# AutoAILab/FusionDepth

Hardware: AMD Instinct MI355X
Metric: training images/sec (640x192, ResNet-18, 4-beam) (higher is better)
Workload: dtype f32

## Files before the change

fusiondepth_amd/csrc/conv_wino.hip:

```cpp
#include "../../include/fdhip.h"
#include "fd_common.h"
#include "conv_fast.h"
#include "conv_limb.h"
#include <stdlib.h>
#include <type_traits>

namespace {

typedef float f32x16 __attribute__((ext_vector_type(16)));
typedef float f32x2 __attribute__((ext_vector_type(2)));
typedef unsigned int u32x2 __attribute__((__vector_size__(2 * sizeof(unsigned int))));

__device__ __forceinline__ f32x2 fd_ldg64(__amdgpu_buffer_rsrc_t r, unsigned byte_off) {
    return __builtin_bit_cast(f32x2, __builtin_amdgcn_raw_buffer_load_b64(r, (int)byte_off, 0, 0));
}
__device__ __attribute__((noinline)) float wino_act_slow(float v, int act) {
    if (act == 2) return v > 0.f ? v : expm1f(v);
    if (act == 3) return 1.0f / (1.0f + expf(-v));
    return tanhf(v);
}
__device__ __forceinline__ float wino_act(float v, int act) {
    if (act >= 2) return wino_act_slow(v, act);
    return act == 1 ? fmaxf(v, 0.f) : v;
}
// ... 1538 lines not shown
            rx[i].z = fmaf(x_sgn, rz[i].z, rx[i].z); rx[i].w = fmaf(x_sgn, rz[i].w, rx[i].w);
        }
        if (!HALFM || i < 2) *reinterpret_cast<f32x2*>(qa) = ra[i];
        const bool L = rf & 1, R = rf & 2;
        float4 d;
        d.y = L ? rx[i].x : rx[i].y;
        d.z = L ? rx[i].y : rx[i].z;
        d.w = L ? rx[i].z : rx[i].w;
        d.x = L ? (refl ? d.z : 0.f) : rx[i].x;
        d.w = R ? (refl ? d.y : 0.f) : d.w;
        *reinterpret_cast<float4*>(smem + buf * WG_BUF_FLOATS + WBM * LDG + (rw + 16 * i) * LDX + 4 * p) = d;
    };

    const int wm = wave >> 1, wn = wave & 1;
    const int arow = lane >> 5, acol = lane & 31;
    f32x16 acc[4];
#pragma unroll
    for (int t = 0; t < 4; ++t)
#pragma unroll
        for (int r = 0; r < 16; ++r) acc[t][r] = 0.f;

    constexpr int NK = WGP / 2, LS = NK / 2;
    constexpr int NKW = HALFM ? NK / 2 : NK;
    static_assert(!HALFM || NKW == LS, "HALFM: the four row loads / stores of a chunk sit in its four k-steps");
    const int kb = HALFM ? wm * NKW : 0;
    if (nchunk > 0) {
        prep_chunk(true);
        rf = pf;
#pragma unroll
        for (int i = 0; i < 4; ++i) load_row(i);
#pragma unroll
        for (int i = 0; i < 4; ++i) store_row(0, i);
        prep_chunk(1 < nchunk);
        rf = pf;
#pragma unroll
        for (int i = 0; i < 4; ++i) load_row(i);
        prep_chunk(2 < nchunk);
        __syncthreads();
        for (int ch = 0; ch < nchunk; ++ch) {
            const int cur = ch & 1;
            const float* pa = smem + cur * WG_BUF_FLOATS + ((HALFM ? 0 : 32 * wm) + acol) * LDG + 2 * arow + 4 * kb;
            const float* pb = smem + cur * WG_BUF_FLOATS + WBM * LDG + (32 * wn + acol) * LDX + 4 * arow + 8 * kb;
            float av[2][4], bv[2][4];
            f32x2 yy;
            float4 dd;
            auto read_ops = [&](int kk2) __attribute__((always_inline)) {
                yy = *reinterpret_cast<const f32x2*>(pa + 4 * kk2);
                dd = *reinterpret_cast<const float4*>(pb + 8 * kk2);
            };
            auto xform = [&](int nb) __attribute__((always_inline)) {
                av[nb][0] = yy.x; av[nb][1] = yy.x + yy.y; av[nb][2] = yy.x - yy.y; av[nb][3] = yy.y;
                bv[nb][0] = dd.x - dd.z; bv[nb][1] = dd.y + dd.z; bv[nb][2] = dd.z - dd.y; bv[nb][3] = dd.y - dd.w;
            };
            read_ops(0); xform(0);
#pragma unroll
            for (int kk = 0; kk < NKW; ++kk) {
                const int cb = kk & 1, nb = cb ^ 1;
                __builtin_amdgcn_sched_barrier(0);
                acc[0] = __builtin_amdgcn_mfma_f32_32x32x2f32(av[cb][0], bv[cb][0], acc[0], 0, 0, 0);
                __builtin_amdgcn_sched_barrier(0);
                if (kk + 1 < NKW) read_ops(kk + 1);
                __builtin_amdgcn_sched_barrier(0);
                acc[1] = __builtin_amdgcn_mfma_f32_32x32x2f32(av[cb][1], bv[cb][1], acc[1], 0, 0, 0);
                __builtin_amdgcn_sched_barrier(0);
                if (kk < LS) store_row(cur ^ 1, kk);
                __builtin_amdgcn_sched_barrier(0);
                acc[2] = __builtin_amdgcn_mfma_f32_32x32x2f32(av[cb][2], bv[cb][2], acc[2], 0, 0, 0);
                __builtin_amdgcn_sched_barrier(0);
                if (kk + 1 < NKW) xform(nb);
                __builtin_amdgcn_sched_barrier(0);
                acc[3] = __builtin_amdgcn_mfma_f32_32x32x2f32(av[cb][3], bv[cb][3], acc[3], 0, 0, 0);
                __builtin_amdgcn_sched_barrier(0);
                if (kk < LS) load_row(kk);
                if (kk == (HALFM ? NKW - 1 : LS)) rf = pf;
                if (kk == NKW - 1) prep_chunk(ch + 3 < nchunk);
            }
            __builtin_amdgcn_sched_barrier(0);
            __syncthreads();
        }
    }

    if constexpr (HALFM) {
        float* red = smem + ((wn * 64) << 6) + lane;
        if (wm == 1) {
#pragma unroll
            for (int t = 0; t < 4; ++t)
#pragma unroll
                for (int r = 0; r < 16; ++r) red[(t * 16 + r) << 6] = acc[t][r];
        }
        __syncthreads();
        if (wm == 1) return;
#pragma unroll
        for (int t = 0; t < 4; ++t)
#pragma unroll
            for (int r = 0; r < 16; ++r) acc[t][r] += red[(t * 16 + r) << 6];
    }
    const int c = c0 + 32 * wn + acol;
    const __amdgpu_buffer_rsrc_t rsS = fd_make_rsrc(g.slabs + (size_t)bs * ((size_t)g.M * (3 * R) * g.C));
    const int mb = m0 + (HALFM ? 0 : 32 * wm) + 4 * arow;
    const unsigned col = (c < g.C) ? 4u * (unsigned)(ky * 3 * g.C + c) : FD_OOB;
    const unsigned row_step = 4u * (3u * R) * (unsigned)g.C, kx_step = 4u * (unsigned)g.C;
#pragma unroll
    for (int r = 0; r < 16; ++r) {
        const int m = mb + (r & 3) + 8 * (r >> 2);
        const unsigned off = (m < g.M) ? col + (unsigned)m * row_step : FD_OOB;
        const float M0 = acc[0][r], M1 = acc[1][r], M2 = acc[2][r], M3 = acc[3][r];
        const float h = 0.5f * (M1 + M2);
        __builtin_amdgcn_raw_buffer_store_b32(__builtin_bit_cast(unsigned, M0 + h), rsS, (int)off, 0, 0);
        __builtin_amdgcn_raw_buffer_store_b32(__builtin_bit_cast(unsigned, 0.5f * (M1 - M2)), rsS, (int)(off + kx_step), 0, 0);
        __builtin_amdgcn_raw_buffer_store_b32(__builtin_bit_cast(unsigned, h - M3), rsS, (int)(off + 2u * kx_step), 0, 0);
    }
}

constexpr int WL_HPL = 64 * 16 + 64;
constexpr int WL_PLANE = 2 * WL_HPL;
constexpr int WL_OP = 12 * WL_PLANE;
constexpr int WL_LDS_BYTES = 2 * WL_OP;


template <bool REFL>
__global__ void __launch_bounds__(WNT) k_wgrad_wino_limb(WinoWgradArgs g) {
    extern __shared__ __attribute__((aligned(16))) float smem[];
    unsigned char* smemb = reinterpret_cast<unsigned char*>(smem);
    const int tid = threadIdx.x, lane = tid & 63;
    const int wave = __builtin_amdgcn_readfirstlane(tid >> 6);
    const int W2 = g.W >> 1;
    const int HT = g.H >> 1;
    constexpr int R = 4;
    const int plane2 = HT * W2, Np = g.Nb * plane2;
    const unsigned hw = (unsigned)(g.H * g.W);
    const int ctiles = (g.C + WBN - 1) / WBN;
    int bt, bs, by;
    if (g.slice_major == 2) {
        const int mtiles = (g.M + WBM - 1) / WBM, nt = R * ctiles * mtiles;
        const int L = blockIdx.x, xcd = L & 7, k = L >> 3;
        int t;
        if (g.xcds_per_slice <= 1) { t = k % nt; bs = (k / nt) * 8 + xcd; }
        else { const int per = nt / g.xcds_per_slice; bs = xcd / g.xcds_per_slice; t = (xcd % g.xcds_per_slice) * per + k; }
        by = t / (R * ctiles);
        bt = t - by * R * ctiles;
    } else {
        bt = g.slice_major ? blockIdx.z : blockIdx.x; bs = g.slice_major ? blockIdx.x : blockIdx.z; by = blockIdx.y;
    }
    const int ky = bt / ctiles, c0 = (bt - ky * ctiles) * WBN;
    const int m0 = by * WBM;
    const int pp_lo = (int)((long)bs * g.pairs_per_split < Np ? (long)bs * g.pairs_per_split : Np);
    const int pp_hi = (long)pp_lo + g.pairs_per_split < Np ? pp_lo + (int)g.pairs_per_split : Np;
    const int nchunk = pp_hi > pp_lo ? (pp_hi - pp_lo + WGP - 1) / WGP : 0;

    const int q = tid & 3, row = tid >> 2;
    unsigned a_row, b_row;
    {
        int m = m0 + row; m = m < g.M ? m : g.M - 1;
        int c = c0 + row; c = c < g.C ? c : g.C - 1;
        a_row = 4u * (unsigned)m * hw; b_row = 4u * (unsigned)c * hw;
    }
    const __amdgpu_buffer_rsrc_t rsY = fd_make_rsrc(g.dY);
    const __amdgpu_buffer_rsrc_t rsX = __builtin_amdgcn_make_buffer_rsrc(const_cast<float*>(g.X), 0, (int)(4u * (unsigned)g.Nb * (unsigned)g.C * hw), 0x00020000);
    float4 ya[1][2], yb[1][2];
    float4 xa[1][2], xb[1][2];
    f32x2 xa2[1], xb2[1];
    unsigned a_off = FD_OOB, x_off = FD_OOB, a_off2 = FD_OOB, x_off2 = FD_OOB;
    const int yr_a = ky == 3 ? 1 : 0;
    const bool y_two = ky == 1 || ky == 2;
    const float y_sgn = ky == 2 ? -1.f : 1.f;
    const int xr_a = ky == 0 ? 0 : (ky == 2 ? 2 : 1), xr_b = ky == 3 ? 3 : (ky == 2 ? 1 : 2);
    const float x_sgn = ky == 1 ? 1.f : -1.f;
    int pf = 0, rf = 0;
    int pc = pp_lo;
    int cn, cy, cj;
    {
        const int pq = pp_lo + 4 * q;
        cn = pq / plane2;
        const int rem = pq - cn * plane2;
        cy = rem / W2; cj = rem - cy * W2;
    }
    auto prep_chunk = [&](bool live) __attribute__((always_inline)) {
        const int pg = pc + 4 * q;
        const bool ok = live & (pg < pp_hi);
        const int n = cn, y = cy, j = cj;
        const bool e_left = j == 0, e_right = 2 * j + 8 >= g.W;
        auto x_row = [&](int r) __attribute__((always_inline)) {
            const bool inb = (unsigned)r < (unsigned)g.H;
            int rr_ = r < 0 ? -r : r;
            rr_ = rr_ >= g.H ? 2 * g.H - 2 - rr_ : rr_;
            const int ruse = REFL ? rr_ : r;
            const bool okb = ok & (REFL | inb);
            const unsigned base = 4u * ((unsigned)n * (unsigned)g.C * hw + (unsigned)(ruse * g.W + 2 * j));
            return okb ? (e_left ? base : base - 4u) : FD_OOB;
        };
        const unsigned yo = 4u * ((unsigned)n * (unsigned)g.M * hw + (unsigned)((2 * y + yr_a) * g.W + 2 * j));
        a_off = ok ? yo : FD_OOB;
        a_off2 = (ok & y_two) ? yo + 4u * (unsigned)g.W : FD_OOB;
        x_off = x_row(2 * y - 1 + xr_a);
        x_off2 = x_row(2 * y - 1 + xr_b);
        pf = (e_left ? 1 : 0) | (e_right ? 2 : 0);
        pc += WGP;
        cj += g.adv_j;
        const bool c1 = cj >= W2;
        cj -= c1 ? W2 : 0;
        cy += g.adv_y + (c1 ? 1 : 0);
        const bool c2 = cy >= HT;
        cy -= c2 ? HT : 0;
        cn += g.adv_n + (c2 ? 1 : 0);
    };
    auto load_all = [&](auto slot_tag) __attribute__((always_inline)) {
        constexpr int S = decltype(slot_tag)::value;
        ya[S][0] = fd_ldg128(rsY, a_off + a_row); ya[S][1] = fd_ldg128(rsY, a_off + a_row + 16u);
        yb[S][0] = fd_ldg128(rsY, a_off2 + a_row); yb[S][1] = fd_ldg128(rsY, a_off2 + a_row + 16u);
        xa[S][0] = fd_ldg128(rsX, x_off + b_row); xa[S][1] = fd_ldg128(rsX, x_off + b_row + 16u); xa2[S] = fd_ldg64(rsX, x_off + b_row + 32u);
        xb[S][0] = fd_ldg128(rsX, x_off2 + b_row); xb[S][1] = fd_ldg128(rsX, x_off2 + b_row + 16u); xb2[S] = fd_ldg64(rsX, x_off2 + b_row + 32u);
    };
    unsigned char* const slot = smemb + (q >> 1) * WL_HPL + row * 16 + 8 * (q & 1);
    auto store_all = [&](auto slot_tag) __attribute__((always_inline)) {
        constexpr int S = decltype(slot_tag)::value;
        float Y[8], X[10];
        Y[0] = fmaf(y_sgn, yb[S][0].x, ya[S][0].x); Y[1] = fmaf(y_sgn, yb[S][0].y, ya[S][0].y); Y[2] = fmaf(y_sgn, yb[S][0].z, ya[S][0].z); Y[3] = fmaf(y_sgn, yb[S][0].w, ya[S][0].w);
        Y[4] = fmaf(y_sgn, yb[S][1].x, ya[S][1].x); Y[5] = fmaf(y_sgn, yb[S][1].y, ya[S][1].y); Y[6] = fmaf(y_sgn, yb[S][1].z, ya[S][1].z); Y[7] = fmaf(y_sgn, yb[S][1].w, ya[S][1].w);
        float r[10];
        r[0] = fmaf(x_sgn, xb[S][0].x, xa[S][0].x); r[1] = fmaf(x_sgn, xb[S][0].y, xa[S][0].y); r[2] = fmaf(x_sgn, xb[S][0].z, xa[S][0].z); r[3] = fmaf(x_sgn, xb[S][0].w, xa[S][0].w);
        r[4] = fmaf(x_sgn, xb[S][1].x, xa[S][1].x); r[5] = fmaf(x_sgn, xb[S][1].y, xa[S][1].y); r[6] = fmaf(x_sgn, xb[S][1].z, xa[S][1].z); r[7] = fmaf(x_sgn, xb[S][1].w, xa[S][1].w);
        r[8] = fmaf(x_sgn, xb2[S].x, xa2[S].x); r[9] = fmaf(x_sgn, xb2[S].y, xa2[S].y);
        const bool L = rf & 1, Rr = rf & 2;
#pragma unroll
        for (int k = 1; k < 10; ++k) X[k] = L ? r[k - 1] : r[k];
        X[0] = L ? (REFL ? X[2] : 0.f) : r[0];
        X[9] = Rr ? (REFL ? X[7] : 0.f) : X[9];
        unsigned char* qa = slot;
        unsigned char* qb = slot + WL_OP;
#pragma unroll
        for (int t = 0; t < 4; ++t) {
            float pv[4], qv[4];
#pragma unroll
            for (int k = 0; k < 4; ++k) {
                const float y0 = Y[2 * k], y1 = Y[2 * k + 1];
                const float d0 = X[2 * k], d1 = X[2 * k + 1], d2 = X[2 * k + 2], d3 = X[2 * k + 3];
                pv[k] = t == 0 ? y0 : (t == 1 ? y0 + y1 : (t == 2 ? y0 - y1 : y1));
                qv[k] = t == 0 ? d0 - d2 : (t == 1 ? d1 + d2 : (t == 2 ? d2 - d1 : d1 - d3));
            }
            unsigned h0, m0_, l0, h1, m1, l1;
            fdlimb::split2(pv[0], pv[1], h0, m0_, l0); fdlimb::split2(pv[2], pv[3], h1, m1, l1);
            *reinterpret_cast<u32x2*>(qa + (3 * t) * WL_PLANE) = u32x2{h0, h1};
            *reinterpret_cast<u32x2*>(qa + (3 * t + 1) * WL_PLANE) = u32x2{m0_, m1};
            *reinterpret_cast<u32x2*>(qa + (3 * t + 2) * WL_PLANE) = u32x2{l0, l1};
            fdlimb::split2(qv[0], qv[1], h0, m0_, l0); fdlimb::split2(qv[2], qv[3], h1, m1, l1);
            *reinterpret_cast<u32x2*>(qb + (3 * t) * WL_PLANE) = u32x2{h0, h1};
            *reinterpret_cast<u32x2*>(qb + (3 * t + 1) * WL_PLANE) = u32x2{m0_, m1};
            *reinterpret_cast<u32x2*>(qb + (3 * t + 2) * WL_PLANE) = u32x2{l0, l1};
        }
    };

    const int wm = wave >> 1, wn = wave & 1;
    const int arow = lane >> 5, acol = lane & 31;
    f32x16 acc[4];
#pragma unroll
    for (int t = 0; t < 4; ++t)
#pragma unroll
        for (int r = 0; r < 16; ++r) acc[t][r] = 0.f;

    if (nchunk > 0) {
        constexpr std::integral_constant<int, 0> S0{};
        prep_chunk(true);
        rf = pf;
        load_all(S0);
        prep_chunk(1 < nchunk);
        const unsigned char* fa = smemb + arow * WL_HPL + (32 * wm + acol) * 16;
        const unsigned char* fb = smemb + WL_OP + arow * WL_HPL + (32 * wn + acol) * 16;
        for (int ch = 0; ch < nchunk; ++ch) {
            store_all(S0);
            __syncthreads();
            load_all(S0);
            rf = pf;
            prep_chunk(ch + 2 < nchunk);
#pragma unroll
            for (int t = 0; t < 4; ++t) {
                uint4 af[3], bf[3];
#pragma unroll
                for (int Lm = 0; Lm < 3; ++Lm) {
                    af[Lm] = *reinterpret_cast<const uint4*>(fa + (t * 3 + Lm) * WL_PLANE);
                    bf[Lm] = *reinterpret_cast<const uint4*>(fb + (t * 3 + Lm) * WL_PLANE);
                }
                FD_WLIMB_MFMA6(acc[t], af, bf);
            }
            __syncthreads();
        }
    }
    const int c = c0 + 32 * wn + acol;
    const __amdgpu_buffer_rsrc_t rsS = fd_make_rsrc(g.slabs + (size_t)bs * ((size_t)g.M * (3 * R) * g.C));
    const int mb = m0 + 32 * wm + 4 * arow;
    const unsigned col = (c < g.C) ? 4u * (unsigned)(ky * 3 * g.C + c) : FD_OOB;
    const unsigned row_step = 4u * (3u * R) * (unsigned)g.C, kx_step = 4u * (unsigned)g.C;
#pragma unroll
    for (int r = 0; r < 16; ++r) {
        const int m = mb + (r & 3) + 8 * (r >> 2);
        const unsigned off = (m < g.M) ? col + (unsigned)m * row_step : FD_OOB;
        const float M0 = acc[0][r], M1 = acc[1][r], M2 = acc[2][r], M3 = acc[3][r];
        const float hh = 0.5f * (M1 + M2);
        __builtin_amdgcn_raw_buffer_store_b32(__builtin_bit_cast(unsigned, M0 + hh), rsS, (int)off, 0, 0);
        __builtin_amdgcn_raw_buffer_store_b32(__builtin_bit_cast(unsigned, 0.5f * (M1 - M2)), rsS, (int)(off + kx_step), 0, 0);
        __builtin_amdgcn_raw_buffer_store_b32(__builtin_bit_cast(unsigned, hh - M3), rsS, (int)(off + 2u * kx_step), 0, 0);
    }
}

inline int wino_splits(const fd_conv_desc* d, int M, int C) {
    const long tiles = (long)fd_cdiv((long)d->N * d->H * (d->W / 2), WBN) * fd_cdiv(M, WBM);
    const int nchunk = 3 * (C / WBKC);
    int sp = 1;
    const long target = fd_tun().wino_target;
    if (tiles < target) {
        sp = (int)(target / tiles);
        const int cap = nchunk / 3 > 0 ? (nchunk / 3 < 16 ? nchunk / 3 : 16) : 1;
        if (sp > cap) sp = cap;
        if (sp < 1) sp = 1;
    }
    return sp;
}

}

bool wino_fwd_ok(const fd_conv_desc* d) {
    return d->KH == 3 && d->KW == 3 && d->stride == 1 && d->pad == 1 && d->Cin % 16 == 0 && d->W % 2 == 0 && !d->in_norm &&
           (long)d->Cout * 3 * d->Cin * 4 * 4 < 2147483648L;
}
int wino_fwd_mode(const fd_conv_desc* d) {
    if (!wino_fwd_ok(d) || d->H % 2 != 0 || (long)d->Cout * 4 * d->Cin * 4 * 4 >= 2147483648L) return 0;
    const fd_tuning& t = fd_tun();
    const long wgs = (long)fd_cdiv((long)d->N * (d->H / 2) * (d->W / 2), WBN) * fd_cdiv(d->Cout, WBM);
    const long cc_min = d->pad_mode == 1 ? (t.wino_fwd_2d_min < 8192 ? t.wino_fwd_2d_min : 8192) : t.wino_fwd_2d_min;
    const bool deep = t.wino_fwd_2d_min > 0 && (long)d->Cin * d->Cout >= cc_min;
    if (t.wino_fwd_2dp_min_wgs > 0 && wgs >= (long)t.wino_fwd_2dp_min_wgs && (!deep || t.wino_fwd_2dp_deep)) return 2;
    return deep ? 1 : 0;
}
bool wino_fwd_2d(const fd_conv_desc* d) { return wino_fwd_mode(d) != 0; }
bool wino_fwd_limb(const fd_conv_desc* d) {
    return fd_tun().wino_fwd_limb != 0 && wino_fwd_mode(d) == 1 && d->Cout >= 64 && d->W % 4 == 0 && d->Cin % 16 == 0 && d->Cin >= 64;
}
inline int wino2d_ksplits_bm(const fd_conv_desc* d, int bm) {
    const long tiles = 4L * fd_cdiv((long)d->N * (d->H / 2) * (d->W / 2), WBN) * fd_cdiv(d->Cout, bm);
    const long target = fd_tun().wino_target;
    long ks = tiles < target ? target / tiles : 1;
    const long cap = d->Cin / WBKC / 4 > 0 ? d->Cin / WBKC / 4 : 1;
    if (ks > cap) ks = cap;
    if (ks > 4) ks = 4;
    return ks < 1 ? 1 : (int)ks;
}
inline bool wino2d_m128(const fd_conv_desc* d) {
    if (fd_tun().wino_fwd_2d_m128 == 0 || d->Cout % M2_BM != 0 || d->W % 4 != 0 || d->Cin % M2_KC != 0) return false;
    if (fd_tun().wino_fwd_2d_m128 != 2) return true;
    const long px = fd_cdiv((long)d->N * (d->H / 2) * (d->W / 2), WBN);
    const long n64 = 4L * px * fd_cdiv(d->Cout, WBM) * wino2d_ksplits_bm(d, WBM), n128 = 4L * px * (d->Cout / M2_BM) * wino2d_ksplits_bm(d, M2_BM);
    const long s64 = 3 * 256, s128 = 2 * 256;
    return n128 * (fd_cdiv(n64, s64) * s64) > n64 * (fd_cdiv(n128, s128) * s128);
}
inline int wino2d_ksplits(const fd_conv_desc* d) { return wino2d_ksplits_bm(d, (!wino_fwd_limb(d) && wino2d_m128(d)) ? M2_BM : WBM); }
long wino_wt_floats(const fd_conv_desc* d) {
    if (wino_fwd_limb(d)) return 24L * d->Cout * d->Cin;
    return 4L * d->Cout * (wino_fwd_2d(d) ? 4 : 3) * d->Cin;
}
long wino_ws_floats(const fd_conv_desc* d) {
    const int mode = wino_fwd_mode(d);
    if (mode == 2) return 0;
    if (mode == 1) return 4L * wino2d_ksplits(d) * d->N * d->Cout * (d->H / 2) * d->W;
    const int sp = wino_splits(d, d->Cout, d->Cin);
    return sp > 1 ? (long)sp * d->N * d->Cout * d->H * d->W : 0;
}
int wino_weight_launch(const fd_conv_desc* d, const float* w, float* U, int flip, hipStream_t st) {
    const int M = d->Cout, C = d->Cin;
    const bool twod = wino_fwd_2d(d);
    if (wino_fwd_limb(d)) {
        const long nl = (long)M * 4 * (C >> 3);
        hipLaunchKernelGGL(k_wino_weight2d_limb, dim3(fd_cdiv(nl, 256) > 4096 ? 4096 : fd_cdiv(nl, 256)), dim3(256), 0, st, w, reinterpret_cast<uint4*>(U), M, C, flip);
        FD_LAUNCH_CHECK("wino weight transform (limbs)");
        return 0;
    }
    const long n = (long)M * (twod ? 4 : 3) * C;
    const dim3 grid(fd_cdiv(n, 256) > 4096 ? 4096 : fd_cdiv(n, 256));
    if (twod) hipLaunchKernelGGL(k_wino_weight2d, grid, dim3(256), 0, st, w, U, M, C, flip);
    else hipLaunchKernelGGL(k_wino_weight, grid, dim3(256), 0, st, w, U, M, C, flip);
    FD_LAUNCH_CHECK("wino weight transform");
    return 0;
}
int wino_stat_slots(const fd_conv_desc* d) {
    if (!wino_fwd_ok(d) || d->act != 0) return 0;
    const int mode = wino_fwd_mode(d);
    if (mode == 1) return 0;
    if (mode == 2) {
        const long tiles = (long)(d->H / 2) * (d->W / 2);
        if (tiles % WBN == 0) return (int)(2 * tiles / WBN);
        return (tiles % 32 == 0 && d->W % 4 == 0 && fd_tun().wino_fwd_2dp_dma != 0) ? (int)(tiles / 32) : 0;
    }
    const long plane2 = (long)d->H * (d->W / 2);
    if (plane2 % WBN != 0 || wino_splits(d, d->Cout, d->Cin) != 1) return 0;
    return (int)(2 * plane2 / WBN);
}

bool wino_fwd_slab_route(const fd_conv_desc* d) { return wino_fwd_ok(d) && wino_fwd_mode(d) == 1; }

int wino_conv_launch(const fd_conv_desc* d, const float* x, const float* U, const float* bias, float* y, float* ws, hipStream_t st,
                     const float* add, float* stat_part, const BnAfterConv* bn) {
    if (bn && (wino_fwd_mode(d) != 1 || bias || add || d->act != 0)) { fd_set_error("wino conv: the fused BatchNorm needs the slab route without bias / activation"); return -1; }
    WinoArgs g = {};
    g.U = U; g.X = x; g.Y = y; g.bias = bias; g.slabs = ws; g.add = add;
    g.stat_part = stat_part; g.stat_slots = stat_part ? wino_stat_slots(d) : 0;
    if (stat_part && g.stat_slots == 0) { fd_set_error("wino conv: no statistics epilogue for this shape"); return -1; }
    g.M = d->Cout; g.C = d->Cin; g.Nb = d->N; g.H = d->H; g.W = d->W;
    g.pad_mode = d->pad_mode; g.act = d->act;
    const long out_total = (long)d->N * d->Cout * d->H * d->W;
    g.slab_stride = out_total;
    const int mode = wino_fwd_mode(d);
    const bool twod = mode == 1;
    const int sp = twod ? 4 * wino2d_ksplits(d) : (mode == 2 ? 1 : wino_splits(d, d->Cout, d->Cin));
    if (sp > 1 && !ws) { fd_set_error("wino conv: split-K workspace missing"); return -1; }
    static FdLdsAttrOnce attr_set;
    if (attr_set.needed()) {
        (void)hipFuncSetAttribute(reinterpret_cast<const void*>(k_conv_wino2d), hipFuncAttributeMaxDynamicSharedMemorySize, 160 * 1024);
        (void)hipFuncSetAttribute(reinterpret_cast<const void*>(k_conv_wino<false, false>), hipFuncAttributeMaxDynamicSharedMemorySize, 160 * 1024);
        (void)hipFuncSetAttribute(reinterpret_cast<const void*>(k_conv_wino<false, true>), hipFuncAttributeMaxDynamicSharedMemorySize, 160 * 1024);
        (void)hipFuncSetAttribute(reinterpret_cast<const void*>(k_conv_wino<true, false>), hipFuncAttributeMaxDynamicSharedMemorySize, 160 * 1024);
        (void)hipFuncSetAttribute(reinterpret_cast<const void*>(k_conv_wino<true, true>), hipFuncAttributeMaxDynamicSharedMemorySize, 160 * 1024);
        (void)hipFuncSetAttribute(reinterpret_cast<const void*>(k_conv_wino2p<false>), hipFuncAttributeMaxDynamicSharedMemorySize, 160 * 1024);
        (void)hipFuncSetAttribute(reinterpret_cast<const void*>(k_conv_wino2p<true>), hipFuncAttributeMaxDynamicSharedMemorySize, 160 * 1024);
        (void)hipFuncSetAttribute(reinterpret_cast<const void*>(k_conv_wino2p_dma<false>), hipFuncAttributeMaxDynamicSharedMemorySize, 160 * 1024);
        (void)hipFuncSetAttribute(reinterpret_cast<const void*>(k_conv_wino2p_dma<true>), hipFuncAttributeMaxDynamicSharedMemorySize, 160 * 1024);
        attr_set.mark();
    }
    if (mode == 2) {
        const long img_tiles = (long)(d->H / 2) * (d->W / 2);
        const bool aligned = stat_part && img_tiles % WBN != 0;
        const int gx2 = aligned ? d->N * fd_cdiv(img_tiles, WBN) : fd_cdiv((long)d->N * img_tiles, WBN), gy2 = fd_cdiv(d->Cout, WBM);
        g.img_tiles = aligned ? fd_cdiv(img_tiles, WBN) : 0;
        g.xcd_swizzle = (gx2 % 8 == 0 && gx2 >= 16) ? 1 : 0;
        const bool vdma = fd_tun().wino_fwd_2dp_dma != 0 && d->W % 4 == 0 && ((uintptr_t)x & 15) == 0;
        if (aligned && !vdma) { fd_set_error("wino conv: the statistics epilogue of this shape needs a 16-byte aligned input"); return -1; }
        if (vdma) {
            if (stat_part) hipLaunchKernelGGL(k_conv_wino2p_dma<true>, dim3(gx2, gy2), dim3(WNT), sizeof(float) * W2D_LDS_FLOATS, st, g);
            else if (d->Cout <= 32 && fd_tun().wino_fwd_halfm != 0) {
                static FdLdsAttrOnce attr_h;
                if (attr_h.needed()) { (void)hipFuncSetAttribute(reinterpret_cast<const void*>(k_conv_wino2p_dma<false, true>), hipFuncAttributeMaxDynamicSharedMemorySize, 160 * 1024); attr_h.mark(); }
                hipLaunchKernelGGL((k_conv_wino2p_dma<false, true>), dim3(gx2, gy2), dim3(WNT), sizeof(float) * W2D_LDS_FLOATS, st, g);
            }
            else hipLaunchKernelGGL(k_conv_wino2p_dma<false>, dim3(gx2, gy2), dim3(WNT), sizeof(float) * W2D_LDS_FLOATS, st, g);
        } else if (stat_part) hipLaunchKernelGGL(k_conv_wino2p<true>, dim3(gx2, gy2), dim3(WNT), sizeof(float) * W_LDS_FLOATS, st, g);
        else hipLaunchKernelGGL(k_conv_wino2p<false>, dim3(gx2, gy2), dim3(WNT), sizeof(float) * W_LDS_FLOATS, st, g);
        FD_LAUNCH_CHECK("k_conv_wino2p");
        return 0;
    }
    if (twod) {
        if (stat_part) { fd_set_error("wino conv: no statistics epilogue for this shape"); return -1; }
        const int HT = d->H / 2;
        const int gx2 = fd_cdiv((long)d->N * HT * (d->W / 2), WBN);
        g.slab_stride = out_total / 2;
        const bool limb2d = wino_fwd_limb(d);
        if (limb2d && ((uintptr_t)x & 15) != 0) { fd_set_error("wino conv: the split-precision slab kernel needs a 16-byte aligned input"); return -1; }
        const bool m128 = !limb2d && wino2d_m128(d) && ((uintptr_t)x & 15) == 0;
        const int gy2 = fd_cdiv(d->Cout, m128 ? M2_BM : WBM);
        const int xmap = 1;
        g.xcd_swizzle = (gx2 % 8 == 0 && gx2 >= 16) ? 1 : 0;
        dim3 grid(gx2, gy2, sp);
        if (xmap && (gy2 * sp) % 8 == 0) { g.xcd_swizzle = 2; g.gx = gx2; g.gy = gy2; g.gz = sp; grid = dim3((unsigned)(gx2 * gy2 * sp)); }
        if (limb2d) {
            static FdLdsAttrOnce attr_l;
            if (attr_l.needed()) { (void)hipFuncSetAttribute(reinterpret_cast<const void*>(k_conv_wino2d_limb), hipFuncAttributeMaxDynamicSharedMemorySize, 160 * 1024); attr_l.mark(); }
            hipLaunchKernelGGL(k_conv_wino2d_limb, grid, dim3(WNT), (size_t)W2L_LDS_BYTES, st, g);
        }
        else if (m128) hipLaunchKernelGGL(k_conv_wino2d_m128, grid, dim3(WNT), sizeof(float) * M2_LDS_FLOATS, st, g);
        else hipLaunchKernelGGL(k_conv_wino2d, grid, dim3(WNT), sizeof(float) * W_LDS_FLOATS, st, g);
        FD_LAUNCH_CHECK("k_conv_wino2d");
        if (bn)
            return bn_small_slabs_launch(ws, g.slab_stride, sp / 4, y, *bn, d->N, d->Cout, d->H, d->W, st);
        const unsigned total2 = (unsigned)(out_total / 4);
        const unsigned blocks = (total2 + 255u) / 256u;
        hipLaunchKernelGGL(k_wino2d_finish, dim3(blocks > 4096u ? 4096u : blocks), dim3(256), 0, st, ws, y, bias, add, total2,
                           g.slab_stride, sp / 4, HT, d->W, d->Cout, d->act);
        FD_LAUNCH_CHECK("k_wino2d_finish");
        return 0;
    }
    const int gx = fd_cdiv((long)d->N * d->H * (d->W / 2), WBN), gy = fd_cdiv(d->Cout, WBM);
    g.xcd_swizzle = (gx % 8 == 0 && gx >= 16) ? 1 : 0;
    const bool vdma = d->W % 4 == 0 && ((uintptr_t)x & 15) == 0;
    const bool stats = g.stat_part != nullptr;
    auto kern = vdma ? (stats ? k_conv_wino<true, true> : k_conv_wino<true, false>) : (stats ? k_conv_wino<false, true> : k_conv_wino<false, false>);
    hipLaunchKernelGGL(kern, dim3(gx, gy, sp), dim3(WNT), sizeof(float) * W_LDS_FLOATS, st, g);
    FD_LAUNCH_CHECK("k_conv_wino");
    if (sp > 1) return fast_splitk_finish_launch(ws, y, bias, out_total, out_total, sp, (long)d->H * d->W, d->Cout, d->act, st, add);
    return 0;
}

extern "C" long fd_conv3x3_wino_wt_floats(const fd_conv_desc* d) { return (d && wino_fwd_ok(d)) ? wino_wt_floats(d) : 0; }
extern "C" long fd_conv3x3_wino_ws_floats(const fd_conv_desc* d) { return (d && wino_fwd_ok(d)) ? wino_ws_floats(d) : 0; }
extern "C" int fd_conv3x3_wino_fwd(const fd_conv_desc* d, const float* x, const float* w, const float* bias, float* y, float* wt,
                                   int wt_ready, float* ws, void* stream) {
    FD_REQUIRE(d && x && w && y && wt, "fd_conv3x3_wino_fwd: NULL argument");
    FD_REQUIRE(wino_fwd_ok(d), "fd_conv3x3_wino_fwd: needs a 3x3 stride-1 pad-1 convolution with Cin %% 16 == 0 and an even width");
    hipStream_t st = (hipStream_t)stream;
    if (!wt_ready)
        if (int rc = wino_weight_launch(d, w, wt, 0, st)) return rc;
    return wino_conv_launch(d, x, wt, bias, y, ws, st);
}

bool wino_wgrad_ok(const fd_conv_desc* d) {
    return d->KH == 3 && d->KW == 3 && d->stride == 1 && d->pad == 1 && d->Cin % 16 == 0 && d->Cin >= 64 && d->Cout >= fd_tun().wino_wgrad_min_cout &&
           d->W % 2 == 0 && !d->in_norm;
}
bool wino_wgrad_2d(const fd_conv_desc* d) {
    const int mode = fd_tun().wino_wgrad_2d;
    return mode != 0 && d->H % 2 == 0 && (d->Cin % 32 == 0 || mode >= 2);
}
int wino_wgrad_splits(const fd_conv_desc* d) {
    const bool twod = wino_wgrad_2d(d);
    const long tiles = (twod ? 4L : 3L) * fd_cdiv(d->Cin, WBN) * fd_cdiv(d->Cout, WBM);
    const long Np = (long)d->N * (twod ? d->H / 2 : d->H) * (d->W / 2);
    const long target = fd_tun().wino_wgrad_target;
    long sp = target / tiles;
    const long maxs = (Np + 4 * WGP - 1) / (4 * WGP);
    if (sp > maxs) sp = maxs;
    if (sp > 512) sp = 512;
    if (sp >= 8) sp &= ~7L;
    if (sp < 1) sp = 1;
    return (int)sp;
}
long wino_wgrad_ws_floats(const fd_conv_desc* d) { return (long)wino_wgrad_splits(d) * d->Cout * (wino_wgrad_2d(d) ? 12 : 9) * d->Cin; }
int wino_wgrad_launch(const fd_conv_desc* d, const float* x, const float* gy, float* gw, float* ws, int accumulate, hipStream_t st) {
    WinoWgradArgs g = {};
    g.dY = gy; g.X = x; g.slabs = ws;
    g.M = d->Cout; g.C = d->Cin; g.Nb = d->N; g.H = d->H; g.W = d->W; g.pad_mode = d->pad_mode;
    const int sp = wino_wgrad_splits(d);
    const bool twod = wino_wgrad_2d(d);
    const int HT = twod ? d->H / 2 : d->H;
    g.slab_rows = twod ? 12 : 9;
    const long Np = (long)d->N * HT * (d->W / 2);
    long pps = (Np + sp - 1) / sp;
    pps = (pps + WGP - 1) / WGP * WGP;
    g.pairs_per_split = pps;
    {
        const int W2 = d->W / 2, plane2 = HT * W2;
        g.adv_n = WGP / plane2;
        const int rem = WGP - g.adv_n * plane2;
        g.adv_y = rem / W2; g.adv_j = rem - g.adv_y * W2;
    }
    static FdLdsAttrOnce attr_set;
    if (attr_set.needed()) {
        (void)hipFuncSetAttribute(reinterpret_cast<const void*>(k_wgrad_wino<false, false>), hipFuncAttributeMaxDynamicSharedMemorySize, 160 * 1024);
        (void)hipFuncSetAttribute(reinterpret_cast<const void*>(k_wgrad_wino<true, false>), hipFuncAttributeMaxDynamicSharedMemorySize, 160 * 1024);
        (void)hipFuncSetAttribute(reinterpret_cast<const void*>(k_wgrad_wino<false, true>), hipFuncAttributeMaxDynamicSharedMemorySize, 160 * 1024);
        (void)hipFuncSetAttribute(reinterpret_cast<const void*>(k_wgrad_wino<true, true>), hipFuncAttributeMaxDynamicSharedMemorySize, 160 * 1024);
        attr_set.mark();
    }
    const int slice_major = 2;
    g.slice_major = slice_major;
    const int nt = (twod ? 4 : 3) * fd_cdiv(d->Cin, WBN);
    const int mt = fd_cdiv(d->Cout, WBM);
    g.xcds_per_slice = 1;
    if (slice_major == 2 && sp % 8 != 0) {
        const int q = (sp == 2 || sp == 4) ? 8 / sp : 0;
        if (q > 0 && (nt * mt) % q == 0 && fd_tun().wino_wgrad_xcd_few != 0) g.xcds_per_slice = q;
        else g.slice_major = 0;
    }
    const dim3 grid = g.slice_major == 2 ? dim3((unsigned)(nt * mt * sp)) : (g.slice_major ? dim3(sp, mt, nt) : dim3(nt, mt, sp));
    const size_t lds = sizeof(float) * WG_LDS_FLOATS;
    const bool halfm = d->Cout <= 32 && fd_tun().wino_wgrad_halfm != 0;
    if (fd_tun().wino_wgrad_limb != 0 && twod && (d->pad_mode == 0 || fd_tun().wino_wgrad_limb >= 2) && d->Cout >= 64 && d->W % 8 == 0) {
        static FdLdsAttrOnce attr_l;
        if (attr_l.needed()) {
            (void)hipFuncSetAttribute(reinterpret_cast<const void*>(k_wgrad_wino_limb<false>), hipFuncAttributeMaxDynamicSharedMemorySize, 160 * 1024);
            (void)hipFuncSetAttribute(reinterpret_cast<const void*>(k_wgrad_wino_limb<true>), hipFuncAttributeMaxDynamicSharedMemorySize, 160 * 1024);
            attr_l.mark();
        }
        if (d->pad_mode == 1) hipLaunchKernelGGL(k_wgrad_wino_limb<true>, grid, dim3(WNT), (size_t)WL_LDS_BYTES, st, g);
        else hipLaunchKernelGGL(k_wgrad_wino_limb<false>, grid, dim3(WNT), (size_t)WL_LDS_BYTES, st, g);
    } else if (halfm) {
        static FdLdsAttrOnce attr_h;
        if (attr_h.needed()) {
            (void)hipFuncSetAttribute(reinterpret_cast<const void*>(k_wgrad_wino<false, false, true>), hipFuncAttributeMaxDynamicSharedMemorySize, 160 * 1024);
            (void)hipFuncSetAttribute(reinterpret_cast<const void*>(k_wgrad_wino<true, false, true>), hipFuncAttributeMaxDynamicSharedMemorySize, 160 * 1024);
            (void)hipFuncSetAttribute(reinterpret_cast<const void*>(k_wgrad_wino<false, true, true>), hipFuncAttributeMaxDynamicSharedMemorySize, 160 * 1024);
            (void)hipFuncSetAttribute(reinterpret_cast<const void*>(k_wgrad_wino<true, true, true>), hipFuncAttributeMaxDynamicSharedMemorySize, 160 * 1024);
            attr_h.mark();
        }
        if (twod) {
            if (d->pad_mode == 1) hipLaunchKernelGGL((k_wgrad_wino<true, true, true>), grid, dim3(WNT), lds, st, g);
            else hipLaunchKernelGGL((k_wgrad_wino<false, true, true>), grid, dim3(WNT), lds, st, g);
        } else {
            if (d->pad_mode == 1) hipLaunchKernelGGL((k_wgrad_wino<true, false, true>), grid, dim3(WNT), lds, st, g);
            else hipLaunchKernelGGL((k_wgrad_wino<false, false, true>), grid, dim3(WNT), lds, st, g);
        }
    } else if (twod) {
        if (d->pad_mode == 1) hipLaunchKernelGGL((k_wgrad_wino<true, true>), grid, dim3(WNT), lds, st, g);
        else hipLaunchKernelGGL((k_wgrad_wino<false, true>), grid, dim3(WNT), lds, st, g);
    } else {
        if (d->pad_mode == 1) hipLaunchKernelGGL((k_wgrad_wino<true, false>), grid, dim3(WNT), lds, st, g);
        else hipLaunchKernelGGL((k_wgrad_wino<false, false>), grid, dim3(WNT), lds, st, g);
    }
    FD_LAUNCH_CHECK("k_wgrad_wino");
    return fast_wgrad_finish_launch(ws, gw, d->Cout, d->Cin, twod ? 12 : 9, sp, accumulate, st);
}
```

Measured before the change: 702.8.

## Add producer/consumer warp-specialized Winograd wgrad limb kernel

Adds a variant of the limb-split Winograd weight-gradient kernel that doubles the workgroup size. Four waves act as producers that load global data, transform it and write limb planes into double-buffered LDS, while four consumer waves run the MFMA accumulation. The aim is to overlap global loads and the transform with matrix math. It is gated behind a tuning value of at least 3, uses twice the LDS, and likely lowers occupancy.

```diff
diff --git a/fusiondepth_amd/csrc/conv_wino.hip b/fusiondepth_amd/csrc/conv_wino.hip
--- a/fusiondepth_amd/csrc/conv_wino.hip
+++ b/fusiondepth_amd/csrc/conv_wino.hip
@@ -1864,6 +1864,214 @@
     }
 }
 
+constexpr int WNT_ROLES = 2 * WNT;
+
+template <bool REFL>
+__global__ void __launch_bounds__(WNT_ROLES) k_wgrad_wino_limb_roles(WinoWgradArgs g) {
+    extern __shared__ __attribute__((aligned(16))) float smem[];
+    unsigned char* smemb = reinterpret_cast<unsigned char*>(smem);
+    const int tid = threadIdx.x & (WNT - 1), lane = tid & 63;
+    const int wave8 = __builtin_amdgcn_readfirstlane((int)threadIdx.x >> 6);
+    const bool producer = wave8 < 4;
+    const int wave = wave8 & 3;
+    const int W2 = g.W >> 1;
+    const int HT = g.H >> 1;
+    constexpr int R = 4;
+    const int plane2 = HT * W2, Np = g.Nb * plane2;
+    const unsigned hw = (unsigned)(g.H * g.W);
+    const int ctiles = (g.C + WBN - 1) / WBN;
+    int bt, bs, by;
+    if (g.slice_major == 2) {
+        const int mtiles = (g.M + WBM - 1) / WBM, nt = R * ctiles * mtiles;
+        const int L = blockIdx.x, xcd = L & 7, k = L >> 3;
+        int t;
+        if (g.xcds_per_slice <= 1) { t = k % nt; bs = (k / nt) * 8 + xcd; }
+        else { const int per = nt / g.xcds_per_slice; bs = xcd / g.xcds_per_slice; t = (xcd % g.xcds_per_slice) * per + k; }
+        by = t / (R * ctiles);
+        bt = t - by * R * ctiles;
+    } else {
+        bt = g.slice_major ? blockIdx.z : blockIdx.x; bs = g.slice_major ? blockIdx.x : blockIdx.z; by = blockIdx.y;
+    }
+    const int ky = bt / ctiles, c0 = (bt - ky * ctiles) * WBN;
+    const int m0 = by * WBM;
+    const int pp_lo = (int)((long)bs * g.pairs_per_split < Np ? (long)bs * g.pairs_per_split : Np);
+    const int pp_hi = (long)pp_lo + g.pairs_per_split < Np ? pp_lo + (int)g.pairs_per_split : Np;
+    const int nchunk = pp_hi > pp_lo ? (pp_hi - pp_lo + WGP - 1) / WGP : 0;
+
+    if (producer) {
+        const int q = tid & 3, row = tid >> 2;
+        unsigned a_row, b_row;
+        {
+            int m = m0 + row; m = m < g.M ? m : g.M - 1;
+            int c = c0 + row; c = c < g.C ? c : g.C - 1;
+            a_row = 4u * (unsigned)m * hw; b_row = 4u * (unsigned)c * hw;
+        }
+        const __amdgpu_buffer_rsrc_t rsY = fd_make_rsrc(g.dY);
+        const __amdgpu_buffer_rsrc_t rsX = __builtin_amdgcn_make_buffer_rsrc(const_cast<float*>(g.X), 0, (int)(4u * (unsigned)g.Nb * (unsigned)g.C * hw), 0x00020000);
+        float4 ya[2][2], yb[2][2];
+        float4 xa[2][2], xb[2][2];
+        f32x2 xa2[2], xb2[2];
+        int rf[2] = {0, 0};
+        unsigned a_off = FD_OOB, x_off = FD_OOB, a_off2 = FD_OOB, x_off2 = FD_OOB;
+        const int yr_a = ky == 3 ? 1 : 0;
+        const bool y_two = ky == 1 || ky == 2;
+        const float y_sgn = ky == 2 ? -1.f : 1.f;
+        const int xr_a = ky == 0 ? 0 : (ky == 2 ? 2 : 1), xr_b = ky == 3 ? 3 : (ky == 2 ? 1 : 2);
+        const float x_sgn = ky == 1 ? 1.f : -1.f;
+        int pf = 0;
+        int pc = pp_lo;
+        int cn, cy, cj;
+        {
+            const int pq = pp_lo + 4 * q;
+            cn = pq / plane2;
+            const int rem = pq - cn * plane2;
+            cy = rem / W2; cj = rem - cy * W2;
+        }
+        auto prep_chunk = [&](bool live) __attribute__((always_inline)) {
+            const int pg = pc + 4 * q;
+            const bool ok = live & (pg < pp_hi);
+            const int n = cn, y = cy, j = cj;
+            const bool e_left = j == 0, e_right = 2 * j + 8 >= g.W;
+            auto x_row = [&](int r) __attribute__((always_inline)) {
+                const bool inb = (unsigned)r < (unsigned)g.H;
+                int rr_ = r < 0 ? -r : r;
+                rr_ = rr_ >= g.H ? 2 * g.H - 2 - rr_ : rr_;
+                const int ruse = REFL ? rr_ : r;
+                const bool okb = ok & (REFL | inb);
+                const unsigned base = 4u * ((unsigned)n * (unsigned)g.C * hw + (unsigned)(ruse * g.W + 2 * j));
+                return okb ? (e_left ? base : base - 4u) : FD_OOB;
+            };
+            const unsigned yo = 4u * ((unsigned)n * (unsigned)g.M * hw + (unsigned)((2 * y + yr_a) * g.W + 2 * j));
+            a_off = ok ? yo : FD_OOB;
+            a_off2 = (ok & y_two) ? yo + 4u * (unsigned)g.W : FD_OOB;
+            x_off = x_row(2 * y - 1 + xr_a);
+            x_off2 = x_row(2 * y - 1 + xr_b);
+            pf = (e_left ? 1 : 0) | (e_right ? 2 : 0);
+            pc += WGP;
+            cj += g.adv_j;
+            const bool c1 = cj >= W2;
+            cj -= c1 ? W2 : 0;
+            cy += g.adv_y + (c1 ? 1 : 0);
+            const bool c2 = cy >= HT;
+            cy -= c2 ? HT : 0;
+            cn += g.adv_n + (c2 ? 1 : 0);
+        };
+        auto load_all = [&](auto slot_tag) __attribute__((always_inline)) {
+            constexpr int S = decltype(slot_tag)::value;
+            ya[S][0] = fd_ldg128(rsY, a_off + a_row); ya[S][1] = fd_ldg128(rsY, a_off + a_row + 16u);
+            yb[S][0] = fd_ldg128(rsY, a_off2 + a_row); yb[S][1] = fd_ldg128(rsY, a_off2 + a_row + 16u);
+            xa[S][0] = fd_ldg128(rsX, x_off + b_row); xa[S][1] = fd_ldg128(rsX, x_off + b_row + 16u); xa2[S] = fd_ldg64(rsX, x_off + b_row + 32u);
+            xb[S][0] = fd_ldg128(rsX, x_off2 + b_row); xb[S][1] = fd_ldg128(rsX, x_off2 + b_row + 16u); xb2[S] = fd_ldg64(rsX, x_off2 + b_row + 32u);
+            rf[S] = pf;
+        };
+        unsigned char* const slot = smemb + (q >> 1) * WL_HPL + row * 16 + 8 * (q & 1);
+        auto store_all = [&](auto slot_tag) __attribute__((always_inline)) {
+            constexpr int S = decltype(slot_tag)::value;
+            float Y[8];
+            Y[0] = fmaf(y_sgn, yb[S][0].x, ya[S][0].x); Y[1] = fmaf(y_sgn, yb[S][0].y, ya[S][0].y); Y[2] = fmaf(y_sgn, yb[S][0].z, ya[S][0].z); Y[3] = fmaf(y_sgn, yb[S][0].w, ya[S][0].w);
+            Y[4] = fmaf(y_sgn, yb[S][1].x, ya[S][1].x); Y[5] = fmaf(y_sgn, yb[S][1].y, ya[S][1].y); Y[6] = fmaf(y_sgn, yb[S][1].z, ya[S][1].z); Y[7] = fmaf(y_sgn, yb[S][1].w, ya[S][1].w);
+            float r[10], X[10];
+            r[0] = fmaf(x_sgn, xb[S][0].x, xa[S][0].x); r[1] = fmaf(x_sgn, xb[S][0].y, xa[S][0].y); r[2] = fmaf(x_sgn, xb[S][0].z, xa[S][0].z); r[3] = fmaf(x_sgn, xb[S][0].w, xa[S][0].w);
+            r[4] = fmaf(x_sgn, xb[S][1].x, xa[S][1].x); r[5] = fmaf(x_sgn, xb[S][1].y, xa[S][1].y); r[6] = fmaf(x_sgn, xb[S][1].z, xa[S][1].z); r[7] = fmaf(x_sgn, xb[S][1].w, xa[S][1].w);
+            r[8] = fmaf(x_sgn, xb2[S].x, xa2[S].x); r[9] = fmaf(x_sgn, xb2[S].y, xa2[S].y);
+            const bool L = rf[S] & 1, Rr = rf[S] & 2;
+#pragma unroll
+            for (int k = 1; k < 10; ++k) X[k] = L ? r[k - 1] : r[k];
+            X[0] = L ? (REFL ? X[2] : 0.f) : r[0];
+            X[9] = Rr ? (REFL ? X[7] : 0.f) : X[9];
+            unsigned char* qa = slot + S * WL_LDS_BYTES;
+            unsigned char* qb = qa + WL_OP;
+#pragma unroll
+            for (int t = 0; t < 4; ++t) {
+                float pv[4], qv[4];
+#pragma unroll
+                for (int k = 0; k < 4; ++k) {
+                    const float y0 = Y[2 * k], y1 = Y[2 * k + 1];
+                    const float d0 = X[2 * k], d1 = X[2 * k + 1], d2 = X[2 * k + 2], d3 = X[2 * k + 3];
+                    pv[k] = t == 0 ? y0 : (t == 1 ? y0 + y1 : (t == 2 ? y0 - y1 : y1));
+                    qv[k] = t == 0 ? d0 - d2 : (t == 1 ? d1 + d2 : (t == 2 ? d2 - d1 : d1 - d3));
+                }
+                unsigned h0, m0_, l0, h1, m1, l1;
+                fdlimb::split2(pv[0], pv[1], h0, m0_, l0); fdlimb::split2(pv[2], pv[3], h1, m1, l1);
+                *reinterpret_cast<u32x2*>(qa + (3 * t) * WL_PLANE) = u32x2{h0, h1};
+                *reinterpret_cast<u32x2*>(qa + (3 * t + 1) * WL_PLANE) = u32x2{m0_, m1};
+                *reinterpret_cast<u32x2*>(qa + (3 * t + 2) * WL_PLANE) = u32x2{l0, l1};
+                fdlimb::split2(qv[0], qv[1], h0, m0_, l0); fdlimb::split2(qv[2], qv[3], h1, m1, l1);
+                *reinterpret_cast<u32x2*>(qb + (3 * t) * WL_PLANE) = u32x2{h0, h1};
+                *reinterpret_cast<u32x2*>(qb + (3 * t + 1) * WL_PLANE) = u32x2{m0_, m1};
+                *reinterpret_cast<u32x2*>(qb + (3 * t + 2) * WL_PLANE) = u32x2{l0, l1};
+            }
+        };
+        constexpr std::integral_constant<int, 0> S0{};
+        constexpr std::integral_constant<int, 1> S1{};
+        if (nchunk > 0) {
+            prep_chunk(true);
+            load_all(S0);
+            prep_chunk(1 < nchunk);
+            load_all(S1);
+            prep_chunk(2 < nchunk);
+            store_all(S0);
+            load_all(S0);
+            prep_chunk(3 < nchunk);
+        }
+        __syncthreads();
+        for (int ch = 0; ch < nchunk; ch += 2) {
+            if (ch + 1 < nchunk) store_all(S1);
+            load_all(S1);
+            prep_chunk(ch + 4 < nchunk);
+            __syncthreads();
+            if (ch + 2 < nchunk) store_all(S0);
+            load_all(S0);
+            prep_chunk(ch + 5 < nchunk);
+            __syncthreads();
+        }
+        return;
+    }
+
+    const int wm = wave >> 1, wn = wave & 1;
+    const int arow = lane >> 5, acol = lane & 31;
+    f32x16 acc[4];
+#pragma unroll
+    for (int t = 0; t < 4; ++t)
+#pragma unroll
+        for (int r = 0; r < 16; ++r) acc[t][r] = 0.f;
+    {
+        const unsigned char* fa = smemb + arow * WL_HPL + (32 * wm + acol) * 16;
+        const unsigned char* fb = smemb + WL_OP + arow * WL_HPL + (32 * wn + acol) * 16;
+        __syncthreads();
+        for (int ch = 0; ch < nchunk; ++ch) {
+            const int cur = (ch & 1) * WL_LDS_BYTES;
+#pragma unroll
+            for (int t = 0; t < 4; ++t) {
+                uint4 af[3], bf[3];
+#pragma unroll
+                for (int Lm = 0; Lm < 3; ++Lm) {
+                    af[Lm] = *reinterpret_cast<const uint4*>(fa + cur + (t * 3 + Lm) * WL_PLANE);
+                    bf[Lm] = *reinterpret_cast<const uint4*>(fb + cur + (t * 3 + Lm) * WL_PLANE);
+                }
+                FD_WLIMB_MFMA6(acc[t], af, bf);
+            }
+            __syncthreads();
+        }
+        if (nchunk & 1) __syncthreads();
+    }
+    const int c = c0 + 32 * wn + acol;
+    const __amdgpu_buffer_rsrc_t rsS = fd_make_rsrc(g.slabs + (size_t)bs * ((size_t)g.M * (3 * R) * g.C));
+    const int mb = m0 + 32 * wm + 4 * arow;
+    const unsigned col = (c < g.C) ? 4u * (unsigned)(ky * 3 * g.C + c) : FD_OOB;
+    const unsigned row_step = 4u * (3u * R) * (unsigned)g.C, kx_step = 4u * (unsigned)g.C;
+#pragma unroll
+    for (int r = 0; r < 16; ++r) {
+        const int m = mb + (r & 3) + 8 * (r >> 2);
+        const unsigned off = (m < g.M) ? col + (unsigned)m * row_step : FD_OOB;
+        const float M0 = acc[0][r], M1 = acc[1][r], M2 = acc[2][r], M3 = acc[3][r];
+        const float hh = 0.5f * (M1 + M2);
+        __builtin_amdgcn_raw_buffer_store_b32(__builtin_bit_cast(unsigned, M0 + hh), rsS, (int)off, 0, 0);
+        __builtin_amdgcn_raw_buffer_store_b32(__builtin_bit_cast(unsigned, 0.5f * (M1 - M2)), rsS, (int)(off + kx_step), 0, 0);
+        __builtin_amdgcn_raw_buffer_store_b32(__builtin_bit_cast(unsigned, hh - M3), rsS, (int)(off + 2u * kx_step), 0, 0);
+    }
+}
+
 inline int wino_splits(const fd_conv_desc* d, int M, int C) {
     const long tiles = (long)fd_cdiv((long)d->N * d->H * (d->W / 2), WBN) * fd_cdiv(M, WBM);
     const int nchunk = 3 * (C / WBKC);
@@ -2126,9 +2334,16 @@
         if (attr_l.needed()) {
             (void)hipFuncSetAttribute(reinterpret_cast<const void*>(k_wgrad_wino_limb<false>), hipFuncAttributeMaxDynamicSharedMemorySize, 160 * 1024);
             (void)hipFuncSetAttribute(reinterpret_cast<const void*>(k_wgrad_wino_limb<true>), hipFuncAttributeMaxDynamicSharedMemorySize, 160 * 1024);
+            (void)hipFuncSetAttribute(reinterpret_cast<const void*>(k_wgrad_wino_limb_roles<false>), hipFuncAttributeMaxDynamicSharedMemorySize, 160 * 1024);
+            (void)hipFuncSetAttribute(reinterpret_cast<const void*>(k_wgrad_wino_limb_roles<true>), hipFuncAttributeMaxDynamicSharedMemorySize, 160 * 1024);
             attr_l.mark();
         }
-        if (d->pad_mode == 1) hipLaunchKernelGGL(k_wgrad_wino_limb<true>, grid, dim3(WNT), (size_t)WL_LDS_BYTES, st, g);
+        const bool roles = fd_tun().wino_wgrad_limb >= 3;
+        if (fd_tun().log) fprintf(stderr, "FDWGRAD wino %s N=%d Cin=%d H=%d W=%d Cout=%d pad_mode=%d slices=%d\n", roles ? "limb roles" : "limb", d->N, d->Cin, d->H, d->W, d->Cout, d->pad_mode, sp);
+        if (roles) {
+            if (d->pad_mode == 1) hipLaunchKernelGGL(k_wgrad_wino_limb_roles<true>, grid, dim3(WNT_ROLES), (size_t)(2 * WL_LDS_BYTES), st, g);
+            else hipLaunchKernelGGL(k_wgrad_wino_limb_roles<false>, grid, dim3(WNT_ROLES), (size_t)(2 * WL_LDS_BYTES), st, g);
+        } else if (d->pad_mode == 1) hipLaunchKernelGGL(k_wgrad_wino_limb<true>, grid, dim3(WNT), (size_t)WL_LDS_BYTES, st, g);
         else hipLaunchKernelGGL(k_wgrad_wino_limb<false>, grid, dim3(WNT), (size_t)WL_LDS_BYTES, st, g);
     } else if (halfm) {
         static FdLdsAttrOnce attr_h;
```

Measured after the change: 692.0. 0.985x the previous value.
